# utiasASRL/mm_masking

Measured on AMD Instinct MI355X. Metric: scan-pairs/s (mask-CNN + 10-iter dICP fwd+bwd), higher is better.
Workload: dtype bf16; 1 GPU; BASELINE configs[2]: train_icp_weights step fwd+bwd, batch=32 per GPU, 10 dICP iters, point-to-plane Huber, dim=2; 400x3360 polar radar -> GO-CFAR + peaks + polar->Cartesian 640x640 -> U-Net (hand-written NHWC bf16 MFMA kernels, fp32 masters) -> dICP (fp32 points, fp64 normal equations) -> rot+trans+mask_pts loss -> Adam; batch_per_gpu=32, global_batch=32, scan_pts_pad=5120, map_pts=20000, map_pts_pad=20480, icp_iters=10, parallelism=dp1, scene_density=survey (SURVEY.md 8d: 3 500-5 000 valid scan points of 5 120)

## Files before the change

mm_masking_amd/csrc/mmk_unet.hip:

```cpp
#include <math.h>
#include <stdlib.h>

#include <algorithm>
#include <type_traits>

#include "mmk_common.h"
#include "mmk_unet_shared.h"

namespace {

using namespace mmku;

__device__ __forceinline__ unsigned cvt_pk_bf16(float lo, float hi)
{
    unsigned r;
    asm("v_cvt_pk_bf16_f32 %0, %1, %2" : "=v"(r) : "v"(lo), "v"(hi));
    return r;
}
__device__ __forceinline__ unsigned pk_relu_bf16(unsigned x)
{
    unsigned r;
    asm("v_pk_max_i16 %0, %1, 0" : "=v"(r) : "v"(x));
    return r;
}
// ... 412 lines not shown
    return __builtin_bit_cast(u32x4, o);
}

__device__ __forceinline__ void lds_barrier()
{
    asm volatile("s_waitcnt lgkmcnt(0)\n\ts_barrier" ::: "memory");
}

__device__ __forceinline__ u32x4 poolg_scale(const u32x4 g, float scale)
{
    float f[8];
    unpack8(g, f);
#pragma unroll
    for (int j = 0; j < 8; ++j) f[j] = f[j] * scale;
    return pack8(f);
}
template <int K>
__device__ __forceinline__ u32x4 poolg_route(const u32x4 v, unsigned code)
{
    const unsigned x = code ^ ((unsigned)(K | 4) * 0x11111111u);
    const unsigned t = x | (x >> 1) | (x >> 2);
    const unsigned te = t << 7, to = t << 3;
    u32x4 o;
#pragma unroll
    for (int j = 0; j < 4; ++j) {
        unsigned m;
        asm("v_pk_ashrrev_i16 %0, %1, %2" : "=v"(m) : "v"(0x000f000fu), "v"(__builtin_amdgcn_perm(to, te, 0x040c000cu + (unsigned)j * 0x01000100u)));
        o[j] = v[j] & ~m;
    }
    return o;
}
__device__ __forceinline__ void poolg_write(bf16 *dst, int pitch, int row, int r0, int c0, int rows, int cols, bool on,
                                            const u32x4 g, unsigned code, float scale)
{
    const u32x4 v = poolg_scale(g, scale);
    const bool r_lo = on && (unsigned)r0 < (unsigned)rows, r_hi = on && (unsigned)(r0 + 1) < (unsigned)rows;
    const bool c_lo = (unsigned)c0 < (unsigned)cols, c_hi = (unsigned)(c0 + 1) < (unsigned)cols;
    if (r_lo && c_lo) *reinterpret_cast<u32x4 *>(dst) = poolg_route<0>(v, code);
    if (r_lo && c_hi) *reinterpret_cast<u32x4 *>(dst + pitch) = poolg_route<1>(v, code);
    if (r_hi && c_lo) *reinterpret_cast<u32x4 *>(dst + row) = poolg_route<2>(v, code);
    if (r_hi && c_hi) *reinterpret_cast<u32x4 *>(dst + row + pitch) = poolg_route<3>(v, code);
}

#ifdef MMK_DEEP_STAMPS
constexpr int MMK_STAMP_STAGES = 24;
__device__ unsigned long long *g_deep_stamp_buf = nullptr;
#define MMK_STAMP(K)                                                                                          \
    do {                                                                                                      \
        if (stamp_stage < MMK_STAMP_STAGES) {                                                                 \
            const unsigned long long t_ = __builtin_amdgcn_s_memtime();                                       \
            if (lane == 0) stamp_lds[(wv * MMK_STAMP_STAGES + stamp_stage) * 8 + (K)] = t_;                    \
        }                                                                                                     \
    } while (0)
#else
#define MMK_STAMP(K) do { } while (0)
#endif

#ifndef MMK_RING_DIAG
#define MMK_RING_DIAG 0
#endif
template <int CK, int CM, int RD, bool EPI, int POOL = 0, bool C8 = false, bool POOLG = false>
__global__ __launch_bounds__(CONV_THREADS) void conv3x3_ring_kernel(const ConvArgs a, int total_tiles, int tiles_per_xcd)
{
    static_assert(!(EPI && POOL), "the pooled output belongs to the forward pass (no epilogue operands)");
    static_assert(!C8 || (CM == 16 && !POOL), "C8: a single output part of exactly 8 channels");
    constexpr int NS = ksteps(CK);
    constexpr int MT = CM / 16;
    constexpr int NT = 4;
    constexpr int PK = lds_pitch(CK);
    constexpr int GPP = CK / 8;
    constexpr int NIN = HT * WT * GPP;
    constexpr int NW = NS * MT * 64;
    constexpr int RIN = (NIN + CONV_THREADS - 1) / CONV_THREADS;
    constexpr int RW = (NW + CONV_THREADS - 1) / CONV_THREADS;
    constexpr int NST = C8 ? 1 : (POOL == 2 ? 2 * MT : MT * NT + (POOL ? MT : 0));
    extern __shared__ __attribute__((aligned(16))) unsigned char smem[];
    bf16 *in_tile = reinterpret_cast<bf16 *>(smem);
    bf16 *w_lds = in_tile + 2 * HT * WT * PK;

    const int tid = threadIdx.x, lane = tid & 63, wv = tid >> 6;
    const int tiles_x = (a.W + TW - 1) / TW, tiles_y = (a.H + TH - 1) / TH;
    const int tpi = tiles_x * tiles_y;
    const int group = blockIdx.y;

    const int xcd = blockIdx.x & 7, nb = gridDim.x >> 3;
    const int t_begin = xcd * tiles_per_xcd;
    const int t_end = (t_begin + tiles_per_xcd < total_tiles) ? t_begin + tiles_per_xcd : total_tiles;
    const int first = t_begin + (blockIdx.x >> 3);
    if (first >= t_end) return;
    const int nt_blk = (t_end - first + nb - 1) / nb;
#ifdef MMK_DEEP_STAMPS
    unsigned long long *stamp_lds = reinterpret_cast<unsigned long long *>(smem + ((size_t)(2 * HT * WT * PK + NS * MT * 512) * sizeof(bf16) + 15) / 16 * 16);
    int stamp_stage = 0;
    for (int i = tid; i < 4 * MMK_STAMP_STAGES * 8; i += CONV_THREADS) stamp_lds[i] = 0ull;
    __syncthreads();
    if (tid == 0) {
        stamp_lds[6] = gridDim.x; stamp_lds[7] = (unsigned long long)nt_blk;
        stamp_lds[8 + 6] = __builtin_amdgcn_s_memtime(); stamp_lds[8 + 7] = __builtin_amdgcn_s_memrealtime();
    }
#endif

    constexpr int PHT = TH / 2 + 2, PWT = TW / 2 + 2, NPIN = PHT * PWT * GPP;
    constexpr int NRIN = POOLG ? (NPIN + CONV_THREADS - 1) / CONV_THREADS : RIN;
    u32x4 rin[RD][NRIN];
    unsigned rcd[POOLG ? RD : 1][POOLG ? NRIN : 1];
    int g_dy[RIN], g_dx[RIN], in_off[RIN];
    bool in_x2[RIN];
#pragma unroll
// ... 1057 lines not shown
            }
        } else {
#pragma unroll
        for (int i = 0; i < RG; ++i) {
            int gi = tv + i * CONV_THREADS;
            gi = gi < NG ? gi : NG - 1;
            const int pix = gi / GPG, gc = gi % GPG;
            const int dy = pix / TW, dx = pix % TW;
            const bool ok = ty0 + dy < a.H && tx0 + dx < a.W;
            const int p = pix0 + dy * a.W + dx;
            const u32x4 *sp = ok ? reinterpret_cast<const u32x4 *>(a.g + ((long)p * a.COUT + group * CM + gc * 8)) : &g_zero16;
            rg[i] = *sp;
        }
        }
    };
    auto store_tile = [&]() {
        int tv = tid;
        asm volatile("" : "+v"(tv));
#pragma unroll
        for (int i = 0; i < RIN; ++i) {
            const int gi = tv + i * CONV_THREADS;
            if (gi < NIN) *reinterpret_cast<u32x4 *>(x_tile + (size_t)(gi / GPP) * PK + (gi % GPP) * 8) = rin[i];
        }
        if constexpr (POOLG) {
#pragma unroll
            for (int i = 0; i < NRG; ++i) {
                const int gi = tv + i * CONV_THREADS;
                const int pp = gi / GPG, gc = gi % GPG;
                const int r0 = 2 * (pp / PWG), c0 = 2 * (pp % PWG);
                poolg_write(g_tile + (r0 * TW + c0) * PG + gc * 8, PG, TW * PG, r0, c0, TH, TW, gi < NPG, rg[i], rc[i], a.g_scale);
            }
        } else {
#pragma unroll
        for (int i = 0; i < RG; ++i) {
            const int gi = tv + i * CONV_THREADS;
            if (gi < NG) *reinterpret_cast<u32x4 *>(g_tile + (size_t)(gi / GPG) * PG + (gi % GPG) * 8) = rg[i];
        }
        }
    };

    int t_first, t_step, t_end;
    if ((gridDim.x & 7) == 0) {
        const int per_xcd = (total_tiles + 7) / 8;
        const int xcd = blockIdx.x & 7;
        t_first = xcd * per_xcd + ((int)blockIdx.x >> 3);
        t_step = (int)gridDim.x >> 3;
        t_end = min(total_tiles, (xcd + 1) * per_xcd);
    } else {
        t_first = blockIdx.x; t_step = gridDim.x; t_end = total_tiles;
    }
    const int adv_tx = t_step % tiles_x, adv_ty = (t_step / tiles_x) % tiles_y, adv_b = t_step / tpi;
    int ld_b = t_first / tpi, ld_ty = (t_first % tpi) / tiles_x, ld_tx = t_first % tiles_x;
    if (t_first < t_end) load_tile(ld_b, ld_ty, ld_tx);
    for (int t = t_first; t < t_end; t += t_step) {
        __syncthreads();
        store_tile();
        __syncthreads();
        {
            if (t + t_step < t_end) {
                ld_tx += adv_tx;
                const int cx = ld_tx >= tiles_x ? 1 : 0;
                ld_tx -= cx ? tiles_x : 0;
                ld_ty += adv_ty + cx;
                const int cy = ld_ty >= tiles_y ? 1 : 0;
                ld_ty -= cy ? tiles_y : 0;
                ld_b += adv_b + cy;
            }
            load_tile(ld_b, ld_ty, ld_tx);
        }
        i32x2 fa[2][2 * MT], fb[2][2 * NTW];
#define WG_ISSUE(R, BUF)                                                                                 \
    {                                                                                                    \
        _Pragma("unroll") for (int m = 0; m < MT; ++m) {                                                 \
            fa[BUF][2 * m] = (m == 0) ? tr_read_o<((R) * TW * PG) * 2>(g_ad)                             \
                           : (m == 1) ? tr_read_o<((R) * TW * PG + 16) * 2>(g_ad)                        \
                           : (m == 2) ? tr_read_o<((R) * TW * PG + 32) * 2>(g_ad)                        \
                                      : tr_read_o<((R) * TW * PG + 48) * 2>(g_ad);                       \
            fa[BUF][2 * m + 1] = (m == 0) ? tr_read_o<((R) * TW * PG + 16 * PG) * 2>(g_ad)                \
                               : (m == 1) ? tr_read_o<((R) * TW * PG + 16 + 16 * PG) * 2>(g_ad)           \
                               : (m == 2) ? tr_read_o<((R) * TW * PG + 32 + 16 * PG) * 2>(g_ad)           \
                                          : tr_read_o<((R) * TW * PG + 48 + 16 * PG) * 2>(g_ad);          \
        }                                                                                                \
        _Pragma("unroll") for (int n = 0; n < NTW; ++n) {                                                \
            fb[BUF][2 * n] = tr_read_o<((R) * WT * PK) * 2>(b_ad[n]);                                    \
            fb[BUF][2 * n + 1] = tr_read_o<((R) * WT * PK + 16 * PK) * 2>(b_ad[n]);                       \
        }                                                                                                \
    }
#define WG_CONSUME(BUF)                                                                                  \
    {                                                                                                    \
        _Pragma("unroll") for (int m = 0; m < MT; ++m) {                                                 \
            const bf16x8 af = frag_from(fa[BUF][2 * m], fa[BUF][2 * m + 1]);                             \
             \
             \
            _Pragma("unroll") for (int n = 0; n < NTW; ++n)                                              \
                acc[m][n] = __builtin_amdgcn_mfma_f32_16x16x32_bf16(af, frag_from(fb[BUF][2 * n], fb[BUF][2 * n + 1]), acc[m][n], 0, 0, 0); \
            accb[m] = __builtin_amdgcn_mfma_f32_16x16x32_bf16(af, ones, accb[m], 0, 0, 0);               \
        }                                                                                                \
    }
#define WG_STEP(R)                                                                                       \
    {                                                                                                    \
        asm volatile("s_waitcnt lgkmcnt(0)" ::: "memory");                                               \
        __builtin_amdgcn_sched_barrier(0);                                                               \
        if ((R) + 1 < TH) WG_ISSUE(((R) + 1 < TH ? (R) + 1 : 0), ((R) + 1) & 1);                         \
        __builtin_amdgcn_sched_barrier(0);                                                               \
        WG_CONSUME((R) & 1);                                                                             \
    }
        WG_ISSUE(0, 0);
        WG_STEP(0) WG_STEP(1) WG_STEP(2) WG_STEP(3) WG_STEP(4) WG_STEP(5) WG_STEP(6) WG_STEP(7)
        static_assert(TH == 8, "WG_STEP expansion above covers 8 tile rows");
#undef WG_STEP
#undef WG_CONSUME
#undef WG_ISSUE
    }

    const size_t pstride = (size_t)9 * a.COUT * a.CIN + a.COUT;
#pragma unroll
    for (int m = 0; m < MT; ++m) {
#pragma unroll
        for (int rr = 0; rr < 4; ++rr) {
            const int co = group * CM + m * 16 + g4 * 4 + rr;
            if (co >= a.COUT) continue;
#pragma unroll
            for (int n = 0; n < NTW; ++n) {
                const int nt = wv + 4 * n;
                if (nt >= NTT) continue;
                int tap, ci;
                if (CK >= 16) {
                    tap = nt / (CK / 16);
                    ci = chunk * CK + (nt % (CK / 16)) * 16 + i16;
                } else {
                    tap = 2 * nt + (i16 >> 3);
                    ci = i16 & 7;
                }
                if (tap < 9) {
                    float *d = a.partials + (size_t)blockIdx.x * pstride + ((size_t)tap * a.COUT + co) * a.CIN + ci;
                    *d = a.acc_partials ? *d + acc[m][n][rr] : acc[m][n][rr];
                }
            }
            if (wv == 0 && chunk == 0 && i16 == 0) {
                float *d = a.partials + (size_t)blockIdx.x * pstride + (size_t)9 * a.COUT * a.CIN + co;
                *d = a.acc_partials ? *d + accb[m][rr] : accb[m][rr];
            }
        }
    }
}

constexpr size_t wgrad_smem(int CX, int CG)
{
    return ((size_t)(HT * WT + 8) * wg_pitch(CX) + (size_t)(TH * TW + 8) * wg_pitch(CG)) * sizeof(bf16);
}

template <int CK, int CM, bool G8>
int wgrad_spatial(int cout, int cin, int B, int H, int W)
{
    constexpr int cap = (CK <= 16 && CM == 16) ? 4 : 8;
    int per_cu = 0;
    if (blocks_per_cu<conv3x3_wgrad_kernel<CK, CM, G8>>(CONV_THREADS, wgrad_smem(CK, G8 ? 8 : CM), cap, &per_cu) != hipSuccess) return -1;
    const int tiles = ((W + TW - 1) / TW) * ((H + TH - 1) / TH) * B;
    const int chunks = cin / CK, groups = (cout + CM - 1) / CM;
    int spatial = (256 * per_cu) / (chunks * groups);
    spatial = spatial < 1 ? 1 : (spatial > tiles ? tiles : spatial);
    return spatial >= 8 ? (spatial & ~7) : spatial;
}

template <int CK, int CM, bool G8, bool POOLG = false>
// ... 334 lines not shown
            float *d = a.partials + (size_t)blockIdx.x * pstride + (size_t)9 * CG * CX + co;
            *d = a.acc_partials ? *d + accb[rr] : accb[rr];
        }
    }
}

constexpr int WGD_THREADS = 512;

template <bool POOLG = false>
__global__ __launch_bounds__(WGD_THREADS) void conv3x3_wgrad_deep_kernel(const WgradArgs a)
{
    constexpr int CK = 64, CM = 64, PK = wg_pitch(64), PG = wg_pitch(64);
    extern __shared__ __attribute__((aligned(16))) unsigned char smem[];
    bf16 *x_tile = reinterpret_cast<bf16 *>(smem);
    bf16 *g_tile = x_tile + (HT * WT + 8) * PK;

    const int tid = threadIdx.x, lane = tid & 63;
    const int wv = __builtin_amdgcn_readfirstlane(tid >> 6);
    const int wm = wv >> 2, wc = wv & 3;
    const int chunk = blockIdx.y, group = blockIdx.z;
    const int tiles_x = (a.W + TW - 1) / TW, tiles_y = (a.H + TH - 1) / TH;
    const int tpi = tiles_x * tiles_y;
    const int total_tiles = tpi * a.B;
    const int i16 = lane & 15, g4 = lane >> 4, q = i16 >> 2, pp = i16 & 3;

    f32x4 acc[3][3][2];
    f32x4 accb[2];
#pragma unroll
    for (int m = 0; m < 2; ++m) {
        accb[m] = (f32x4){0.f, 0.f, 0.f, 0.f};
#pragma unroll
        for (int ty = 0; ty < 3; ++ty)
#pragma unroll
            for (int tx = 0; tx < 3; ++tx) acc[ty][tx][m] = (f32x4){0.f, 0.f, 0.f, 0.f};
    }
    bf16x8 ones;
#pragma unroll
    for (int j = 0; j < 8; ++j) ones[j] = (bf16)1.0f;

    const unsigned xb0 = lds_addr(x_tile) + (unsigned)(((4 * g4 + q) * PK + wc * 16 + 4 * pp) * 2);
    const unsigned gb0 = lds_addr(g_tile) + (unsigned)(((4 * g4 + q) * PG + wm * 32 + 4 * pp) * 2);

    constexpr int GPP = CK / 8;
    constexpr int NIN = HT * WT * GPP;
    constexpr int RIN = (NIN + WGD_THREADS - 1) / WGD_THREADS;
    constexpr int GPG = CM / 8;
    constexpr int NG = TH * TW * GPG;
    constexpr int RG = (NG + WGD_THREADS - 1) / WGD_THREADS;
    constexpr int PWG = TW / 2, NPG = (TH / 2) * PWG * GPG;
    constexpr int NRG = POOLG ? (NPG + WGD_THREADS - 1) / WGD_THREADS : RG;
    u32x4 rin[RIN], rg[NRG];
    unsigned rc[POOLG ? NRG : 1];
    const int Hp = a.H >> 1, Wp = a.W >> 1;
    auto load_tile = [&](int b, int tyi, int txi) {
        int tv = tid;
        asm volatile("" : "+v"(tv));
        const int tx0 = txi * TW, ty0 = tyi * TH;
        const int c0 = chunk * CK;
        const bool in1 = c0 < a.C1;
        const bf16 *xb = in1 ? a.x1 : a.x2;
        const int xc = in1 ? a.C1 : a.C2, cb = in1 ? c0 : c0 - a.C1;
#pragma unroll
        for (int i = 0; i < RIN; ++i) {
            int gi = tv + i * WGD_THREADS;
            gi = gi < NIN ? gi : NIN - 1;
            const int pix = gi / GPP, gc = gi % GPP;
            const int yy = ty0 + pix / WT - 1, xx = tx0 + pix % WT - 1;
            const bool ok = yy >= 0 && yy < a.H && xx >= 0 && xx < a.W;
            const size_t p = ((size_t)b * a.H + yy) * a.W + xx;
            const u32x4 *sp = ok ? reinterpret_cast<const u32x4 *>(xb + p * xc + cb + gc * 8) : &g_zero16;
            rin[i] = *sp;
        }
        if constexpr (POOLG) {
#pragma unroll
            for (int i = 0; i < NRG; ++i) {
                int gi = tv + i * WGD_THREADS;
                gi = gi < NPG ? gi : NPG - 1;
                const int pp = gi / GPG, gc = gi % GPG;
                const int py = (ty0 >> 1) + pp / PWG, px = (tx0 >> 1) + pp % PWG;
                const bool ok = py < Hp && px < Wp;
                const size_t e = (((size_t)b * Hp + py) * Wp + px) * (a.COUT >> 3) + ((group * CM) >> 3) + gc;
                rg[i] = *(ok ? reinterpret_cast<const u32x4 *>(a.g + e * 8) : &g_zero16);
                rc[i] = *(ok ? a.g_arg + e : reinterpret_cast<const unsigned *>(&g_zero16));
            }
        } else {
#pragma unroll
        for (int i = 0; i < RG; ++i) {
            int gi = tv + i * WGD_THREADS;
            gi = gi < NG ? gi : NG - 1;
            const int pix = gi / GPG, gc = gi % GPG;
            const int yy = ty0 + pix / TW, xx = tx0 + pix % TW;
            const bool ok = yy < a.H && xx < a.W;
            const size_t p = ((size_t)b * a.H + yy) * a.W + xx;
            const u32x4 *sp = ok ? reinterpret_cast<const u32x4 *>(a.g + p * a.COUT + group * CM + gc * 8) : &g_zero16;
            rg[i] = *sp;
        }
        }
    };
    auto store_tile = [&]() {
        int tv = tid;
        asm volatile("" : "+v"(tv));
#pragma unroll
        for (int i = 0; i < RIN; ++i) {
            const int gi = tv + i * WGD_THREADS;
            if (gi < NIN) *reinterpret_cast<u32x4 *>(x_tile + (size_t)(gi / GPP) * PK + (gi % GPP) * 8) = rin[i];
        }
        if constexpr (POOLG) {
#pragma unroll
            for (int i = 0; i < NRG; ++i) {
                const int gi = tv + i * WGD_THREADS;
                const int pp = gi / GPG, gc = gi % GPG;
                const int r0 = 2 * (pp / PWG), c0 = 2 * (pp % PWG);
                poolg_write(g_tile + (r0 * TW + c0) * PG + gc * 8, PG, TW * PG, r0, c0, TH, TW, gi < NPG, rg[i], rc[i], a.g_scale);
            }
        } else {
#pragma unroll
        for (int i = 0; i < RG; ++i) {
            const int gi = tv + i * WGD_THREADS;
            if (gi < NG) *reinterpret_cast<u32x4 *>(g_tile + (size_t)(gi / GPG) * PG + (gi % GPG) * 8) = rg[i];
        }
        }
    };

    int t_first, t_step, t_end;
    if ((gridDim.x & 7) == 0) {
        const int per_xcd = (total_tiles + 7) / 8;
        const int xcd = blockIdx.x & 7;
        t_first = xcd * per_xcd + ((int)blockIdx.x >> 3);
        t_step = (int)gridDim.x >> 3;
        t_end = min(total_tiles, (xcd + 1) * per_xcd);
    } else {
        t_first = blockIdx.x; t_step = gridDim.x; t_end = total_tiles;
    }
    const int adv_tx = t_step % tiles_x, adv_ty = (t_step / tiles_x) % tiles_y, adv_b = t_step / tpi;
    int ld_b = t_first / tpi, ld_ty = (t_first % tpi) / tiles_x, ld_tx = t_first % tiles_x;
    if (t_first < t_end) load_tile(ld_b, ld_ty, ld_tx);
    for (int t = t_first; t < t_end; t += t_step) {
        __syncthreads();
        store_tile();
        __syncthreads();
        {
            if (t + t_step < t_end) {
                ld_tx += adv_tx;
                const int cx = ld_tx >= tiles_x ? 1 : 0;
                ld_tx -= cx ? tiles_x : 0;
                ld_ty += adv_ty + cx;
                const int cy = ld_ty >= tiles_y ? 1 : 0;
                ld_ty -= cy ? tiles_y : 0;
                ld_b += adv_b + cy;
            }
            load_tile(ld_b, ld_ty, ld_tx);
        }
        i32x2 fb[2][3][2], fa[4][2][2];
#define WGD_ISSUE(RHO)                                                                                   \
    {                                                                                                    \
        fb[(RHO) & 1][0][0] = tr_read_o<(((RHO) * WT + 0) * PK) * 2>(xb0);                               \
        fb[(RHO) & 1][0][1] = tr_read_o<(((RHO) * WT + 0) * PK + 16 * PK) * 2>(xb0);                     \
        fb[(RHO) & 1][1][0] = tr_read_o<(((RHO) * WT + 1) * PK) * 2>(xb0);                               \
        fb[(RHO) & 1][1][1] = tr_read_o<(((RHO) * WT + 1) * PK + 16 * PK) * 2>(xb0);                     \
        fb[(RHO) & 1][2][0] = tr_read_o<(((RHO) * WT + 2) * PK) * 2>(xb0);                               \
        fb[(RHO) & 1][2][1] = tr_read_o<(((RHO) * WT + 2) * PK + 16 * PK) * 2>(xb0);                     \
        if ((RHO) < TH) {                                                                                \
            constexpr int R_ = (RHO) < TH ? (RHO) : 0;                                                   \
            fa[R_ & 3][0][0] = tr_read_o<((R_ * TW) * PG) * 2>(gb0);                                     \
            fa[R_ & 3][0][1] = tr_read_o<((R_ * TW) * PG + 16 * PG) * 2>(gb0);                           \
            fa[R_ & 3][1][0] = tr_read_o<((R_ * TW) * PG + 16) * 2>(gb0);                                \
            fa[R_ & 3][1][1] = tr_read_o<((R_ * TW) * PG + 16 + 16 * PG) * 2>(gb0);                      \
        }                                                                                                \
    }
#define WGD_STEP(RHO)                                                                                    \
    {                                                                                                    \
        asm volatile("s_waitcnt lgkmcnt(0)" ::: "memory");                                               \
        __builtin_amdgcn_sched_barrier(0);                                                               \
                                          \
        if ((RHO) + 1 < HT) WGD_ISSUE(((RHO) + 1 < HT ? (RHO) + 1 : 0));                                 \
        __builtin_amdgcn_sched_barrier(0);                                                               \
        bf16x8 bfr[3];                                                                                   \
        _Pragma("unroll") for (int tx = 0; tx < 3; ++tx) bfr[tx] = frag_from(fb[(RHO) & 1][tx][0], fb[(RHO) & 1][tx][1]); \
        _Pragma("unroll") for (int ty = 0; ty < 3; ++ty) {                                               \
            const int r = (RHO) - ty;                \
            if (r >= 0 && r < TH) {                                                                      \
                _Pragma("unroll") for (int m = 0; m < 2; ++m) {                                          \
                    const bf16x8 af = frag_from(fa[r & 3][m][0], fa[r & 3][m][1]);                       \
                    _Pragma("unroll") for (int tx = 0; tx < 3; ++tx)                                     \
                        acc[ty][tx][m] = __builtin_amdgcn_mfma_f32_16x16x32_bf16(af, bfr[tx], acc[ty][tx][m], 0, 0, 0); \
                    if (ty == 0) accb[m] = __builtin_amdgcn_mfma_f32_16x16x32_bf16(af, ones, accb[m], 0, 0, 0);  \
                }                                                                                        \
            }                                                                                            \
        }                                                                                                \
        __builtin_amdgcn_sched_barrier(0);                                                               \
    }
        WGD_ISSUE(0);
        WGD_STEP(0) WGD_STEP(1) WGD_STEP(2) WGD_STEP(3) WGD_STEP(4)
        WGD_STEP(5) WGD_STEP(6) WGD_STEP(7) WGD_STEP(8) WGD_STEP(9)
        static_assert(HT == 10, "WGD_STEP expansion above covers 10 halo rows");
#undef WGD_STEP
#undef WGD_ISSUE
    }

    const size_t pstride = (size_t)9 * a.COUT * a.CIN + a.COUT;
#pragma unroll
    for (int m = 0; m < 2; ++m) {
#pragma unroll
        for (int rr = 0; rr < 4; ++rr) {
            const int co = group * CM + (wm * 2 + m) * 16 + g4 * 4 + rr;
            const int ci = chunk * CK + wc * 16 + i16;
            {
                float *ps = a.partials + (size_t)blockIdx.x * pstride + (size_t)co * a.CIN + ci;
#pragma unroll
                for (int ty = 0; ty < 3; ++ty)
#pragma unroll
                    for (int tx = 0; tx < 3; ++tx) {
                        float *d = ps + (size_t)(ty * 3 + tx) * a.COUT * a.CIN;
                        *d = a.acc_partials ? *d + acc[ty][tx][m][rr] : acc[ty][tx][m][rr];
                    }
            }
            if (wc == 0 && chunk == 0 && i16 == 0) {
                float *d = a.partials + (size_t)blockIdx.x * pstride + (size_t)9 * a.COUT * a.CIN + co;
                *d = a.acc_partials ? *d + accb[m][rr] : accb[m][rr];
            }
        }
    }
}

int wgrad_deep_slices(int cout, int cin, int B, int H, int W)
{
    const int tiles = ((W + TW - 1) / TW) * ((H + TH - 1) / TH) * B;
    const int chunks = cin / 64, groups = cout / 64;
    int spatial = 256 / (chunks * groups);
    spatial = spatial < 1 ? 1 : (spatial > tiles ? tiles : spatial);
    return spatial >= 8 ? (spatial & ~7) : spatial;
}

bool wgrad_is_deep(int cout, int cin, int c1) { return cin % 64 == 0 && cout % 64 == 0 && c1 % 64 == 0; }

template <bool POOLG = false>
int launch_wgrad_deep(const WgradArgs &a, hipStream_t st)
{
    constexpr size_t smem = wgrad_smem(64, 64);
    MMK_CHECK_HIP(raise_lds_limit<conv3x3_wgrad_deep_kernel<POOLG>>(true, smem));
    const int spatial = wgrad_deep_slices(a.COUT, a.CIN, a.B, a.H, a.W);
    const int chunks = a.CIN / 64, groups = a.COUT / 64;
    hipLaunchKernelGGL(conv3x3_wgrad_deep_kernel<POOLG>, dim3(spatial, chunks, groups), dim3(WGD_THREADS), smem, st, a);
    MMK_LAUNCH_CHECK();
    return MMK_OK;
}

template <class F>
int with_wgrad_shape(int cout, int cin, F &&f)
{
    return with_int<8, 16, 32, 64>(cin_chunk(cin), [&](auto K) {
        return with_int<16, 32, 64>(cout_group(cout), [&](auto M) {
            if constexpr (M() == 16) {
                if (cout == 8) return f(K, M, std::true_type{});
            }
            return f(K, M, std::false_type{});
        });
    });
}

int dispatch_wgrad(const WgradArgs &a, hipStream_t st)
{
    if (a.g_arg != nullptr) {
        if (wgrad_is_deep(a.COUT, a.CIN, a.C1)) return launch_wgrad_deep<true>(a, st);
        if (a.CIN == 32 && a.COUT == 32) return launch_wgrad<32, 32, false, true>(a, st);
        mmk::set_error("mmk_conv3x3_wgrad_partial_pooled: unsupported channel counts CIN=%d COUT=%d", a.CIN, a.COUT);
        return MMK_ERR_ARG;
    }
    if (wgrad_is_deep(a.COUT, a.CIN, a.C1)) return launch_wgrad_deep(a, st);
    const int rc = with_wgrad_shape(a.COUT, a.CIN, [&](auto K, auto M, auto G8) { return launch_wgrad<K(), M(), G8()>(a, st); });
    if (rc != NO_KERNEL) return rc;
    mmk::set_error("mmk_conv3x3_wgrad: unsupported channel counts CIN=%d COUT=%d", a.CIN, a.COUT);
    return MMK_ERR_ARG;
}

int wgrad_slices(int cout, int cin, int c1, int B, int H, int W)
{
    if (wgrad_is_deep(cout, cin, c1)) return wgrad_deep_slices(cout, cin, B, H, W);
    const int ns = with_wgrad_shape(cout, cin, [&](auto K, auto M, auto G8) { return wgrad_spatial<K(), M(), G8()>(cout, cin, B, H, W); });
    return ns == NO_KERNEL ? 0 : ns;
}

struct UnpackBatch {
    const float *src[PACK_BATCH_MAX];
    float *dW[PACK_BATCH_MAX];
    float *db[PACK_BATCH_MAX];
    int cout[PACK_BATCH_MAX], cin[PACK_BATCH_MAX], slices[PACK_BATCH_MAX];
};

__host__ __device__ inline int unpack_groups(int total) { return total < 8192 ? 16 : (total < 65536 ? 4 : 1); }

__global__ __launch_bounds__(256) void unpack_wgrad_batch_kernel(const UnpackBatch ub)
// ... 255 lines not shown
#pragma unroll
            for (int px = 0; px < 4; ++px) {
                bf16x8 o;
#pragma unroll
                for (int co = 0; co < 8; ++co) o[co] = (bf16)(LK ? act_leaky(acc[px][co], slope) : fmaxf(acc[px][co], 0.f));
                *reinterpret_cast<bf16x8 *>(dst + px * 8) = o;
            }
#pragma unroll
            for (int dy = 0; dy < 3; ++dy)
#pragma unroll
                for (int i = 0; i < 6; ++i) rv[dy][i] = rn[dy][i];
            mv = mn;
        }
        return;
    }
    for (int e = blockIdx.x * blockDim.x + threadIdx.x; e < nq; e += gridDim.x * blockDim.x) {
        const int q = e % Wq, by = e / Wq;
        const int yy = by % H, b = by / H;
        const int x0 = q * 4;
        float acc[4][8];
#pragma unroll
        for (int px = 0; px < 4; ++px)
#pragma unroll
            for (int co = 0; co < 8; ++co) acc[px][co] = bs[co];
        for (int c = 0; c < CIN; ++c) {
            const float *xc = x + ((size_t)b * CIN + c) * H * W;
            const float psub = pre ? pre[2 * c] : 0.f, prcp = pre ? pre[2 * c + 1] : 1.f;
#pragma unroll
            for (int dy = 0; dy < 3; ++dy) {
                float v[6];
                load_row6(xc, yy + dy - 1, x0, H, W, psub, prcp, v);
#pragma unroll
                for (int co = 0; co < 8; ++co) {
#pragma unroll
                    for (int tx = 0; tx < 3; ++tx) {
                        const float w = Wt[(co * CIN + c) * 9 + dy * 3 + tx];
#pragma unroll
                        for (int px = 0; px < 4; ++px) acc[px][co] = __builtin_fmaf(v[px + tx], w, acc[px][co]);
                    }
                }
            }
        }
        bf16 *dst = y + ((size_t)by * W + x0) * 8;
#pragma unroll
        for (int px = 0; px < 4; ++px) {
            bf16x8 o;
#pragma unroll
            for (int co = 0; co < 8; ++co) o[co] = (bf16)(LK ? act_leaky(acc[px][co], slope) : fmaxf(acc[px][co], 0.f));
            *reinterpret_cast<bf16x8 *>(dst + px * 8) = o;
        }
    }
}

__global__ __launch_bounds__(256) void conv_first_wgrad_x4_kernel(const float *__restrict__ x, int CIN, const bf16 *__restrict__ g,
                                                                  const float *__restrict__ pre, int B, int H, int W,
                                                                  float *__restrict__ part )
{
    __shared__ float red[4][80];
    const int lane = threadIdx.x & 63, wv = threadIdx.x >> 6;
    const int Wq = W >> 2;
    const int nq = B * H * Wq;
    const int stride = gridDim.x * blockDim.x;
    for (int c = 0; c < CIN; ++c) {
        const float psub = pre ? pre[2 * c] : 0.f, prcp = pre ? pre[2 * c + 1] : 1.f;
        float acc[80];
#pragma unroll
        for (int i = 0; i < 80; ++i) acc[i] = 0.f;
        bf16x8 gv[4], gn[4];
        float rv[3][6], rn[3][6];
        unsigned mv = 0, mn = 0;
        auto fetch = [&](int e, bf16x8 (&go)[4], float (&ro)[3][6], unsigned &mo) {
            const int q = e % Wq, by = e / Wq;
            const int yy = by % H, b = by / H;
            const int x0 = q * 4;
            const float *xc = x + ((size_t)b * CIN + c) * H * W;
            const bf16 *gp = g + ((size_t)by * W + x0) * 8;
#pragma unroll
            for (int px = 0; px < 4; ++px) go[px] = *reinterpret_cast<const bf16x8 *>(gp + px * 8);
            unsigned m = 0;
#pragma unroll
            for (int dy = 0; dy < 3; ++dy) {
                const int y2 = yy + dy - 1;
                const bool rok = y2 >= 0 && y2 < H;
                const float *row = xc + (size_t)(rok ? y2 : yy) * W;
                const bool lok = x0 > 0, hok = x0 + 4 < W;
                const float4 mid = *reinterpret_cast<const float4 *>(row + x0);
                ro[dy][0] = row[lok ? x0 - 1 : x0];
                ro[dy][1] = mid.x; ro[dy][2] = mid.y; ro[dy][3] = mid.z; ro[dy][4] = mid.w;
                ro[dy][5] = row[hok ? x0 + 4 : x0 + 3];
                m |= (rok ? ((lok ? 1u : 0u) | 0x1Eu | (hok ? 0x20u : 0u)) : 0u) << (6 * dy);
            }
            mo = m;
        };
        int e = blockIdx.x * blockDim.x + threadIdx.x;
        if (e < nq) fetch(e, gv, rv, mv);
        for (; e < nq; e += stride) {
            const int en = e + stride;
            fetch(en < nq ? en : e, gn, rn, mn);
            float v[3][6];
#pragma unroll
            for (int dy = 0; dy < 3; ++dy)
#pragma unroll
                for (int i = 0; i < 6; ++i) {
                    const float t = (rv[dy][i] - psub) * prcp;
                    v[dy][i] = ((mv >> (6 * dy + i)) & 1u) ? (float)(bf16)t : 0.f;
                }
// ... 1290 lines not shown
        const int nblk = (int)std::min<int64_t>(BN_BLOCKS, (npix + per - 1) / per);
        hipLaunchKernelGGL(bn_bwd_reduce_kernel, dim3(nblk), dim3(256), 0, st, (const bf16 *)gd, (const bf16 *)d, drop_scale,
                           (const bf16 *)a, (size_t)npix, C, stat, part);
        MMK_LAUNCH_CHECK();
        hipLaunchKernelGGL(bn_bwd_finalize_kernel, dim3((C + 63) / 64), dim3(64), 0, st, part, nblk, C, (double)npix, gamma, stat,
                           accumulate, coef, dgamma, dbeta);
        MMK_LAUNCH_CHECK();
    } else {
        MMK_REQUIRE(affine != nullptr, "mmk_bn_backward: evaluation mode needs the affine (scale, shift) pairs");
        hipLaunchKernelGGL(bn_eval_coef_kernel, dim3((C + 63) / 64), dim3(64), 0, st, affine, C, coef);
        MMK_LAUNCH_CHECK();
    }
    hipLaunchKernelGGL(bn_bwd_apply_kernel, dim3(gb), dim3(256), 0, st, (const bf16 *)gd, (const bf16 *)d, drop_scale, (const bf16 *)a,
                       ngran, C, stat, coef, leaky_slope, (bf16 *)gz);
    MMK_LAUNCH_CHECK();
    return MMK_OK;
}

static unsigned nblk(size_t n, int t) { return (unsigned)((n + t - 1) / t); }

extern "C" int mmk_channel_minmax(const float *x, int32_t B, int32_t C, int64_t hw, float *part, float *pre, float *minmax,
                                  void *stream)
{
    MMK_REQUIRE(x && part && pre && B >= 1 && C >= 1 && C <= 65535 && hw >= 1, "mmk_channel_minmax: bad argument");
    hipStream_t st = (hipStream_t)stream;
    hipLaunchKernelGGL(channel_minmax_partial_kernel, dim3(MM_BLOCKS, C), dim3(256), 0, st, x, B, C, (size_t)hw, part);
    MMK_LAUNCH_CHECK();
    hipLaunchKernelGGL(channel_minmax_final_kernel, dim3(C), dim3(256), 0, st, part, C, pre, minmax);
    MMK_LAUNCH_CHECK();
    return MMK_OK;
}

extern "C" int mmk_channel_meanstd(const float *x, int32_t B, int32_t C, int64_t hw, double *part, float *pre, void *stream)
{
    MMK_REQUIRE(x && part && pre && B >= 1 && C >= 1 && C <= 65535 && hw >= 1, "mmk_channel_meanstd: bad argument");
    hipStream_t st = (hipStream_t)stream;
    hipLaunchKernelGGL(channel_moment_partial_kernel<false>, dim3(MM_BLOCKS, C), dim3(256), 0, st, x, B, C, (size_t)hw, part);
    MMK_LAUNCH_CHECK();
    hipLaunchKernelGGL(channel_moment_partial_kernel<true>, dim3(MM_BLOCKS, C), dim3(256), 0, st, x, B, C, (size_t)hw, part);
    MMK_LAUNCH_CHECK();
    hipLaunchKernelGGL(channel_meanstd_final_kernel, dim3(C), dim3(256), 0, st, (const double *)part, (size_t)B * (size_t)hw, pre);
    MMK_LAUNCH_CHECK();
    return MMK_OK;
}

extern "C" int mmk_conv_first(const float *x, int32_t cin, const float *W, const float *bias, const float *pre, int32_t B,
                              int32_t H, int32_t Wd, float leaky_slope, void *y, void *stream)
{
    MMK_REQUIRE(x && W && y, "mmk_conv_first: NULL pointer");
    MMK_REQUIRE(leaky_slope >= 0.f && leaky_slope < 1.f, "mmk_conv_first: leaky_slope must be in [0, 1)");
    MMK_REQUIRE(cin >= 1 && cin <= 4 && B >= 1 && H >= 1 && Wd >= 1, "mmk_conv_first: bad shape (cin must be 1..4)");
    const size_t npix = (size_t)B * H * Wd;
    if (Wd % 4 == 0 && npix < (1u << 31)) {
        const unsigned blocks = (unsigned)std::min<size_t>((npix / 4 + 255) / 256, 4096);
        if (leaky_slope > 0.f)
            hipLaunchKernelGGL(conv_first_x4_kernel<true>, dim3(blocks), dim3(256), 0, (hipStream_t)stream, x, cin, W, bias, pre, B, H, Wd,
                               leaky_slope, (bf16 *)y);
        else
            hipLaunchKernelGGL(conv_first_x4_kernel<false>, dim3(blocks), dim3(256), 0, (hipStream_t)stream, x, cin, W, bias, pre, B, H, Wd,
                               leaky_slope, (bf16 *)y);
        MMK_LAUNCH_CHECK();
        return MMK_OK;
    }
    const unsigned blocks = (unsigned)std::min<size_t>((npix + 255) / 256, 8192);
    hipLaunchKernelGGL(conv_first_kernel, dim3(blocks), dim3(256), 0, (hipStream_t)stream, x, cin, W, bias, pre, B, H, Wd, leaky_slope,
                       (bf16 *)y);
    MMK_LAUNCH_CHECK();
    return MMK_OK;
}

extern "C" size_t mmk_conv_first_wgrad_ws_bytes(int32_t cin) { return (size_t)1024 * (cin < 1 ? 1 : cin) * 80 * sizeof(float); }

extern "C" int mmk_conv_first_wgrad(const float *x, int32_t cin, const void *g, const float *pre, int32_t B, int32_t H,
                                    int32_t Wd, float *dW, float *db, float *ws, size_t ws_bytes, void *stream)
{
    MMK_REQUIRE(x && g && dW && ws, "mmk_conv_first_wgrad: NULL pointer");
    MMK_REQUIRE(cin >= 1 && cin <= 4 && B >= 1 && H >= 1 && Wd >= 1, "mmk_conv_first_wgrad: bad shape");
    MMK_REQUIRE(ws_bytes >= mmk_conv_first_wgrad_ws_bytes(cin), "mmk_conv_first_wgrad: workspace too small (%zu < %zu bytes)", ws_bytes,
                mmk_conv_first_wgrad_ws_bytes(cin));
    const size_t npix = (size_t)B * H * Wd;
    unsigned blocks;
    if (Wd % 4 == 0 && npix < (1u << 31)) {
        blocks = (unsigned)std::min<size_t>((npix / 4 + 255) / 256, 512);
        hipLaunchKernelGGL(conv_first_wgrad_x4_kernel, dim3(blocks), dim3(256), 0, (hipStream_t)stream, x, cin, (const bf16 *)g, pre,
                           B, H, Wd, ws);
    } else {
        blocks = (unsigned)std::min<size_t>((npix + 255) / 256, 1024);
        hipLaunchKernelGGL(conv_first_wgrad_kernel, dim3(blocks), dim3(256), 0, (hipStream_t)stream, x, cin, (const bf16 *)g, pre, B,
                           H, Wd, ws);
    }
    MMK_LAUNCH_CHECK();
    hipLaunchKernelGGL(conv_first_wgrad_reduce_kernel, dim3(cin), dim3(320), 0, (hipStream_t)stream, ws, (int)blocks, cin, dW, db);
    MMK_LAUNCH_CHECK();
    return MMK_OK;
}

extern "C" size_t mmk_conv_first_dgrad_ws_bytes(int32_t cin)
{
    return (size_t)(cin < 1 ? 1 : cin) * 4 * (1 + DG_BLOCKS) * sizeof(double);
}

namespace {
template <int CIN, int MODE>
void launch_first_dgrad(bool tiled, unsigned blocks, hipStream_t st, const bf16 *g, const float *W, const float *x, const float *pre,
                        const float *minmax, int B, int H, int Wd, float *gx, double *part)
{
// ... 227 lines not shown
```

Before: 3422 pairs/s.

## Interleave deep wgrad next-tile global loads with the MFMA row steps

The deep weight-gradient kernel's next-tile prefetch no longer issues every global load in one block right after the barrier. Each load is now issued one at a time inside the per-halo-row MFMA steps, with precomputed tile base pointers and unsigned 32-bit address math. The aim is to spread memory traffic across the compute loop, hide latency, and cut address-calculation overhead. The change also adds stamp-based timing instrumentation behind MMK_DEEP_STAMPS, which is compiled out by default, and the tail guards now fold at compile time.

```diff
diff --git a/mm_masking_amd/csrc/mmk_unet.hip b/mm_masking_amd/csrc/mmk_unet.hip
--- a/mm_masking_amd/csrc/mmk_unet.hip
+++ b/mm_masking_amd/csrc/mmk_unet.hip
@@ -488,8 +488,16 @@
             if (lane == 0) stamp_lds[(wv * MMK_STAMP_STAGES + stamp_stage) * 8 + (K)] = t_;                    \
         }                                                                                                     \
     } while (0)
+#define MMK_STAMP_G(K)                                                                                        \
+    do {                                                                                                      \
+        if (stamp_on && stamp_stage < MMK_STAMP_STAGES) {                                                     \
+            const unsigned long long t_ = __builtin_amdgcn_s_memtime();                                       \
+            if (lane == 0) g_deep_stamp_buf[((size_t)(blockIdx.x * 8 + wv) * MMK_STAMP_STAGES + stamp_stage) * 8 + (K)] = t_; \
+        }                                                                                                     \
+    } while (0)
 #else
 #define MMK_STAMP(K) do { } while (0)
+#define MMK_STAMP_G(K) do { } while (0)
 #endif
 
 #ifndef MMK_RING_DIAG
@@ -1653,10 +1661,22 @@
     const int adv_tx = t_step % tiles_x, adv_ty = (t_step / tiles_x) % tiles_y, adv_b = t_step / tpi;
     int ld_b = t_first / tpi, ld_ty = (t_first % tpi) / tiles_x, ld_tx = t_first % tiles_x;
     if (t_first < t_end) load_tile(ld_b, ld_ty, ld_tx);
+#ifdef MMK_DEEP_STAMPS
+    const bool stamp_on = g_deep_stamp_buf != nullptr && blockIdx.x < 64 && blockIdx.y == 0 && blockIdx.z == 0;
+    int stamp_stage = 0;
+#endif
     for (int t = t_first; t < t_end; t += t_step) {
+        MMK_STAMP_G(0);
         __syncthreads();
+        MMK_STAMP_G(1);
+#ifdef MMK_DEEP_STAMPS
+        asm volatile("s_waitcnt vmcnt(0)" ::: "memory");
+#endif
+        MMK_STAMP_G(2);
         store_tile();
+        MMK_STAMP_G(3);
         __syncthreads();
+        MMK_STAMP_G(4);
         {
             if (t + t_step < t_end) {
                 ld_tx += adv_tx;
@@ -1669,6 +1689,7 @@
             }
             load_tile(ld_b, ld_ty, ld_tx);
         }
+        MMK_STAMP_G(5);
         i32x2 fa[2][2 * MT], fb[2][2 * NTW];
 #define WG_ISSUE(R, BUF)                                                                                 \
     {                                                                                                    \
@@ -1707,11 +1728,17 @@
         WG_CONSUME((R) & 1);                                                                             \
     }
         WG_ISSUE(0, 0);
-        WG_STEP(0) WG_STEP(1) WG_STEP(2) WG_STEP(3) WG_STEP(4) WG_STEP(5) WG_STEP(6) WG_STEP(7)
+        WG_STEP(0)
+        MMK_STAMP_G(6);
+        WG_STEP(1) WG_STEP(2) WG_STEP(3) WG_STEP(4) WG_STEP(5) WG_STEP(6) WG_STEP(7)
         static_assert(TH == 8, "WG_STEP expansion above covers 8 tile rows");
 #undef WG_STEP
 #undef WG_CONSUME
 #undef WG_ISSUE
+        MMK_STAMP_G(7);
+#ifdef MMK_DEEP_STAMPS
+        ++stamp_stage;
+#endif
     }
 
     const size_t pstride = (size_t)9 * a.COUT * a.CIN + a.COUT;
@@ -2152,49 +2179,61 @@
     u32x4 rin[RIN], rg[NRG];
     unsigned rc[POOLG ? NRG : 1];
     const int Hp = a.H >> 1, Wp = a.W >> 1;
-    auto load_tile = [&](int b, int tyi, int txi) {
-        int tv = tid;
+    constexpr int NLD = RIN + (POOLG ? 2 * NRG : RG);
+    static_assert(NLD <= HT, "one prefetch load per row step");
+    const int c0 = chunk * CK;
+    const bool in1 = c0 < a.C1;
+    const bf16 *xb = in1 ? a.x1 : a.x2;
+    const int xc = in1 ? a.C1 : a.C2, cb = in1 ? c0 : c0 - a.C1;
+    const bf16 *ld_x = nullptr, *ld_g = nullptr;
+    const unsigned *ld_c = nullptr;
+    int ld_ty0 = 0, ld_tx0 = 0;
+    typedef const __attribute__((address_space(1))) u32x4 *gvec_p;
+    typedef const __attribute__((address_space(1))) unsigned *gword_p;
+    gvec_p zero16 = (gvec_p)&g_zero16;
+    asm volatile("" : "+s"(zero16));
+    auto set_tile = [&](int b, int tyi, int txi) {
+        ld_tx0 = txi * TW;
+        ld_ty0 = tyi * TH;
+        ld_x = xb + (((long)b * a.H + ld_ty0 - 1) * a.W + ld_tx0 - 1) * xc + cb;
+        if constexpr (POOLG) {
+            const long e = (((long)b * Hp + (ld_ty0 >> 1)) * Wp + (ld_tx0 >> 1)) * (a.COUT >> 3) + ((group * CM) >> 3);
+            ld_g = a.g + e * 8;
+            ld_c = a.g_arg + e;
+        } else {
+            ld_g = a.g + (((long)b * a.H + ld_ty0) * a.W + ld_tx0) * a.COUT + group * CM;
+        }
+    };
+    auto issue_load = [&](int j) {
+        unsigned tv = (unsigned)tid;
         asm volatile("" : "+v"(tv));
-        const int tx0 = txi * TW, ty0 = tyi * TH;
-        const int c0 = chunk * CK;
-        const bool in1 = c0 < a.C1;
-        const bf16 *xb = in1 ? a.x1 : a.x2;
-        const int xc = in1 ? a.C1 : a.C2, cb = in1 ? c0 : c0 - a.C1;
-#pragma unroll
-        for (int i = 0; i < RIN; ++i) {
-            int gi = tv + i * WGD_THREADS;
-            gi = gi < NIN ? gi : NIN - 1;
-            const int pix = gi / GPP, gc = gi % GPP;
-            const int yy = ty0 + pix / WT - 1, xx = tx0 + pix % WT - 1;
-            const bool ok = yy >= 0 && yy < a.H && xx >= 0 && xx < a.W;
-            const size_t p = ((size_t)b * a.H + yy) * a.W + xx;
-            const u32x4 *sp = ok ? reinterpret_cast<const u32x4 *>(xb + p * xc + cb + gc * 8) : &g_zero16;
-            rin[i] = *sp;
-        }
-        if constexpr (POOLG) {
-#pragma unroll
-            for (int i = 0; i < NRG; ++i) {
-                int gi = tv + i * WGD_THREADS;
-                gi = gi < NPG ? gi : NPG - 1;
-                const int pp = gi / GPG, gc = gi % GPG;
-                const int py = (ty0 >> 1) + pp / PWG, px = (tx0 >> 1) + pp % PWG;
-                const bool ok = py < Hp && px < Wp;
-                const size_t e = (((size_t)b * Hp + py) * Wp + px) * (a.COUT >> 3) + ((group * CM) >> 3) + gc;
-                rg[i] = *(ok ? reinterpret_cast<const u32x4 *>(a.g + e * 8) : &g_zero16);
-                rc[i] = *(ok ? a.g_arg + e : reinterpret_cast<const unsigned *>(&g_zero16));
-            }
+        if (j < RIN) {
+            unsigned gi = tv + (unsigned)(j * WGD_THREADS);
+            gi = gi < (unsigned)NIN ? gi : (unsigned)(NIN - 1);
+            const unsigned pix = gi / GPP, gc = gi % GPP;
+            const unsigned row = pix / WT, col = pix % WT;
+            const bool ok = ((unsigned)(ld_ty0 - 1) + row < (unsigned)a.H) & ((unsigned)(ld_tx0 - 1) + col < (unsigned)a.W);
+            const unsigned off = (row * (unsigned)a.W + col) * (unsigned)xc + gc * 8;
+            rin[j] = *(ok ? (gvec_p)(ld_x + off) : zero16);
+        } else if constexpr (POOLG) {
+            const int i = (j - RIN) % NRG;
+            unsigned gi = tv + (unsigned)(i * WGD_THREADS);
+            gi = gi < (unsigned)NPG ? gi : (unsigned)(NPG - 1);
+            const unsigned pp = gi / GPG, gc = gi % GPG;
+            const unsigned pr = pp / PWG, pc = pp % PWG;
+            const bool ok = ((unsigned)(ld_ty0 >> 1) + pr < (unsigned)Hp) & ((unsigned)(ld_tx0 >> 1) + pc < (unsigned)Wp);
+            const unsigned e = (pr * (unsigned)Wp + pc) * (unsigned)(a.COUT >> 3) + gc;
+            if (j - RIN < NRG) rg[i] = *(ok ? (gvec_p)(ld_g + e * 8) : zero16);
+            else rc[i] = *(ok ? (gword_p)(ld_c + e) : (gword_p)zero16);
         } else {
-#pragma unroll
-        for (int i = 0; i < RG; ++i) {
-            int gi = tv + i * WGD_THREADS;
-            gi = gi < NG ? gi : NG - 1;
-            const int pix = gi / GPG, gc = gi % GPG;
-            const int yy = ty0 + pix / TW, xx = tx0 + pix % TW;
-            const bool ok = yy < a.H && xx < a.W;
-            const size_t p = ((size_t)b * a.H + yy) * a.W + xx;
-            const u32x4 *sp = ok ? reinterpret_cast<const u32x4 *>(a.g + p * a.COUT + group * CM + gc * 8) : &g_zero16;
-            rg[i] = *sp;
-        }
+            const int i = j - RIN;
+            unsigned gi = tv + (unsigned)(i * WGD_THREADS);
+            gi = gi < (unsigned)NG ? gi : (unsigned)(NG - 1);
+            const unsigned pix = gi / GPG, gc = gi % GPG;
+            const unsigned row = pix / TW, col = pix % TW;
+            const bool ok = ((unsigned)ld_ty0 + row < (unsigned)a.H) & ((unsigned)ld_tx0 + col < (unsigned)a.W);
+            const unsigned off = (row * (unsigned)a.W + col) * (unsigned)a.COUT + gc * 8;
+            rg[i] = *(ok ? (gvec_p)(ld_g + off) : zero16);
         }
     };
     auto store_tile = [&]() {
@@ -2203,7 +2242,7 @@
 #pragma unroll
         for (int i = 0; i < RIN; ++i) {
             const int gi = tv + i * WGD_THREADS;
-            if (gi < NIN) *reinterpret_cast<u32x4 *>(x_tile + (size_t)(gi / GPP) * PK + (gi % GPP) * 8) = rin[i];
+            if ((i + 1) * WGD_THREADS <= NIN || gi < NIN) *reinterpret_cast<u32x4 *>(x_tile + (size_t)(gi / GPP) * PK + (gi % GPP) * 8) = rin[i];
         }
         if constexpr (POOLG) {
 #pragma unroll
@@ -2211,13 +2250,14 @@
                 const int gi = tv + i * WGD_THREADS;
                 const int pp = gi / GPG, gc = gi % GPG;
                 const int r0 = 2 * (pp / PWG), c0 = 2 * (pp % PWG);
-                poolg_write(g_tile + (r0 * TW + c0) * PG + gc * 8, PG, TW * PG, r0, c0, TH, TW, gi < NPG, rg[i], rc[i], a.g_scale);
+                poolg_write(g_tile + (r0 * TW + c0) * PG + gc * 8, PG, TW * PG, r0, c0, TH, TW, (i + 1) * WGD_THREADS <= NPG || gi < NPG, rg[i],
+                            rc[i], a.g_scale);
             }
         } else {
 #pragma unroll
         for (int i = 0; i < RG; ++i) {
             const int gi = tv + i * WGD_THREADS;
-            if (gi < NG) *reinterpret_cast<u32x4 *>(g_tile + (size_t)(gi / GPG) * PG + (gi % GPG) * 8) = rg[i];
+            if ((i + 1) * WGD_THREADS <= NG || gi < NG) *reinterpret_cast<u32x4 *>(g_tile + (size_t)(gi / GPG) * PG + (gi % GPG) * 8) = rg[i];
         }
         }
     };
@@ -2234,11 +2274,29 @@
     }
     const int adv_tx = t_step % tiles_x, adv_ty = (t_step / tiles_x) % tiles_y, adv_b = t_step / tpi;
     int ld_b = t_first / tpi, ld_ty = (t_first % tpi) / tiles_x, ld_tx = t_first % tiles_x;
-    if (t_first < t_end) load_tile(ld_b, ld_ty, ld_tx);
+    if (t_first < t_end) {
+        set_tile(ld_b, ld_ty, ld_tx);
+#pragma unroll
+        for (int j = 0; j < NLD; ++j) issue_load(j);
+    }
+#ifdef MMK_DEEP_STAMPS
+    unsigned long long *stamp_lds = reinterpret_cast<unsigned long long *>(smem + (wgrad_smem(64, 64) + 15) / 16 * 16);
+    int stamp_stage = 0;
+    for (int i = tid; i < 8 * MMK_STAMP_STAGES * 8; i += WGD_THREADS) stamp_lds[i] = 0ull;
+    __syncthreads();
+#endif
     for (int t = t_first; t < t_end; t += t_step) {
+        MMK_STAMP(0);
         __syncthreads();
+        MMK_STAMP(1);
+#ifdef MMK_DEEP_STAMPS
+        asm volatile("s_waitcnt vmcnt(0)" ::: "memory");
+#endif
+        MMK_STAMP(2);
         store_tile();
+        MMK_STAMP(3);
         __syncthreads();
+        MMK_STAMP(4);
         {
             if (t + t_step < t_end) {
                 ld_tx += adv_tx;
@@ -2249,8 +2307,9 @@
                 ld_ty -= cy ? tiles_y : 0;
                 ld_b += adv_b + cy;
             }
-            load_tile(ld_b, ld_ty, ld_tx);
-        }
+            set_tile(ld_b, ld_ty, ld_tx);
+        }
+        MMK_STAMP(5);
         i32x2 fb[2][3][2], fa[4][2][2];
 #define WGD_ISSUE(RHO)                                                                                   \
     {                                                                                                    \
@@ -2275,6 +2334,9 @@
                                           \
         if ((RHO) + 1 < HT) WGD_ISSUE(((RHO) + 1 < HT ? (RHO) + 1 : 0));                                 \
         __builtin_amdgcn_sched_barrier(0);                                                               \
+                                                                                \
+        if ((RHO) < NLD) issue_load((RHO) < NLD ? (RHO) : 0);                                            \
+        __builtin_amdgcn_sched_barrier(0x38F);                                                           \
         bf16x8 bfr[3];                                                                                   \
         _Pragma("unroll") for (int tx = 0; tx < 3; ++tx) bfr[tx] = frag_from(fb[(RHO) & 1][tx][0], fb[(RHO) & 1][tx][1]); \
         _Pragma("unroll") for (int ty = 0; ty < 3; ++ty) {                                               \
@@ -2284,19 +2346,32 @@
                     const bf16x8 af = frag_from(fa[r & 3][m][0], fa[r & 3][m][1]);                       \
                     _Pragma("unroll") for (int tx = 0; tx < 3; ++tx)                                     \
                         acc[ty][tx][m] = __builtin_amdgcn_mfma_f32_16x16x32_bf16(af, bfr[tx], acc[ty][tx][m], 0, 0, 0); \
-                    if (ty == 0) accb[m] = __builtin_amdgcn_mfma_f32_16x16x32_bf16(af, ones, accb[m], 0, 0, 0);  \
+                     \
+                    if (ty == 0) accb[m] = __builtin_amdgcn_mfma_f32_16x16x32_bf16(af, ones, accb[m], 0, 0, 0); \
                 }                                                                                        \
             }                                                                                            \
         }                                                                                                \
         __builtin_amdgcn_sched_barrier(0);                                                               \
     }
         WGD_ISSUE(0);
-        WGD_STEP(0) WGD_STEP(1) WGD_STEP(2) WGD_STEP(3) WGD_STEP(4)
+        WGD_STEP(0)
+        MMK_STAMP(6);
+        WGD_STEP(1) WGD_STEP(2) WGD_STEP(3) WGD_STEP(4)
         WGD_STEP(5) WGD_STEP(6) WGD_STEP(7) WGD_STEP(8) WGD_STEP(9)
         static_assert(HT == 10, "WGD_STEP expansion above covers 10 halo rows");
 #undef WGD_STEP
 #undef WGD_ISSUE
-    }
+        MMK_STAMP(7);
+#ifdef MMK_DEEP_STAMPS
+        ++stamp_stage;
+#endif
+    }
+#ifdef MMK_DEEP_STAMPS
+    __syncthreads();
+    if (g_deep_stamp_buf != nullptr && blockIdx.y == 0 && blockIdx.z == 0 && blockIdx.x < 64)
+        for (int i = tid; i < 8 * MMK_STAMP_STAGES * 8; i += WGD_THREADS)
+            g_deep_stamp_buf[(size_t)blockIdx.x * (8 * MMK_STAMP_STAGES * 8) + i] = stamp_lds[i];
+#endif
 
     const size_t pstride = (size_t)9 * a.COUT * a.CIN + a.COUT;
 #pragma unroll
@@ -2337,7 +2412,11 @@
 template <bool POOLG = false>
 int launch_wgrad_deep(const WgradArgs &a, hipStream_t st)
 {
+#ifdef MMK_DEEP_STAMPS
+    constexpr size_t smem = (wgrad_smem(64, 64) + 15) / 16 * 16 + (size_t)8 * MMK_STAMP_STAGES * 8 * sizeof(unsigned long long);
+#else
     constexpr size_t smem = wgrad_smem(64, 64);
+#endif
     MMK_CHECK_HIP(raise_lds_limit<conv3x3_wgrad_deep_kernel<POOLG>>(true, smem));
     const int spatial = wgrad_deep_slices(a.COUT, a.CIN, a.B, a.H, a.W);
     const int chunks = a.CIN / 64, groups = a.COUT / 64;
```

Result: faster. 3467 pairs/s, median of 6 (+1.3%).

## Add row-band first-conv kernel with sliding window and LDS-transposed coalesced stores

Applied to the files above, without the earlier changes.

Adds a specialised first-convolution kernel for the single-channel, ReLU case. Each thread walks a vertical band of 8 rows with a sliding 3-row register window, so each input row is loaded once instead of three times. Output is reshuffled through a swizzled LDS buffer within each wavefront so global bf16x8 stores become contiguous across lanes. It is on by default with an environment opt-out, and it launches one thread per band-column, which means fewer threads and more serial work per thread.

```diff
diff --git a/mm_masking_amd/csrc/mmk_unet.hip b/mm_masking_amd/csrc/mmk_unet.hip
--- a/mm_masking_amd/csrc/mmk_unet.hip
+++ b/mm_masking_amd/csrc/mmk_unet.hip
@@ -2699,6 +2699,108 @@
     }
 }
 
+constexpr int CF_BAND = 8;
+
+__global__ __launch_bounds__(256) void conv_first_band_kernel(const float *__restrict__ x, const float *__restrict__ Wt,
+                                                              const float *__restrict__ bias, const float *__restrict__ pre, int B,
+                                                              int H, int W, bf16 *__restrict__ y)
+{
+    __shared__ u32x4 xch[4][256];
+    float bs[8];
+#pragma unroll
+    for (int co = 0; co < 8; ++co) bs[co] = bias ? bias[co] : 0.f;
+    const float psub = pre ? pre[0] : 0.f, prcp = pre ? pre[1] : 1.f;
+    const int lane = threadIdx.x & 63, wv = threadIdx.x >> 6;
+    const int Wq = W >> 2;
+    const int nb = (H + CF_BAND - 1) / CF_BAND;
+    const int n_items = B * nb * Wq;
+    const int item_raw = blockIdx.x * blockDim.x + threadIdx.x;
+    const bool valid = item_raw < n_items;
+    const int item = valid ? item_raw : n_items - 1;
+    const int q = item % Wq, t = item / Wq;
+    const int band = t % nb, b = t / nb;
+    const int x0 = q * 4;
+    const int y0 = band * CF_BAND;
+    const int my_rows = valid ? min(H, y0 + CF_BAND) - y0 : 0;
+    const int my_pix = (b * H + y0) * W + x0;
+    int own_pix[4], own_rows[4];
+#pragma unroll
+    for (int k = 0; k < 4; ++k) {
+        own_pix[k] = __shfl(my_pix, k * 16 + (lane >> 2), 64) + (lane & 3);
+        own_rows[k] = __shfl(my_rows, k * 16 + (lane >> 2), 64);
+    }
+    const float *xc = x + (size_t)b * H * W;
+    const bool lok = x0 > 0, hok = x0 + 4 < W;
+    auto fetch = [&](int y2, float (&ro)[6]) {
+        const float *row = xc + (size_t)min(max(y2, 0), H - 1) * W;
+        const float4 mid = *reinterpret_cast<const float4 *>(row + x0);
+        ro[0] = row[lok ? x0 - 1 : x0];
+        ro[1] = mid.x; ro[2] = mid.y; ro[3] = mid.z; ro[4] = mid.w;
+        ro[5] = row[hok ? x0 + 4 : x0 + 3];
+    };
+    auto finish = [&](int y2, const float (&ro)[6], float (&v)[6]) {
+        const bool rok = y2 >= 0 && y2 < H;
+#pragma unroll
+        for (int i = 0; i < 6; ++i) {
+            const float tv = (ro[i] - psub) * prcp;
+            const bool ok = rok && (i != 0 || lok) && (i != 5 || hok);
+            v[i] = ok ? (float)(bf16)tv : 0.f;
+        }
+    };
+    float win[3][6], raw[6];
+    fetch(y0 - 1, raw);
+    finish(y0 - 1, raw, win[0]);
+    fetch(y0, raw);
+    finish(y0, raw, win[1]);
+    fetch(y0 + 1, raw);
+    for (int s = 0; s < CF_BAND; ++s) {
+        if (__ballot(s < my_rows) == 0) break;
+        const int yy = y0 + s;
+        finish(yy + 1, raw, win[2]);
+        fetch(yy + 2, raw);
+        float acc[4][8];
+#pragma unroll
+        for (int px = 0; px < 4; ++px)
+#pragma unroll
+            for (int co = 0; co < 8; ++co) acc[px][co] = bs[co];
+#pragma unroll
+        for (int dy = 0; dy < 3; ++dy)
+#pragma unroll
+            for (int co = 0; co < 8; ++co)
+#pragma unroll
+                for (int tx = 0; tx < 3; ++tx) {
+                    const float w = Wt[co * 9 + dy * 3 + tx];
+#pragma unroll
+                    for (int px = 0; px < 4; ++px) acc[px][co] = __builtin_fmaf(win[dy][px + tx], w, acc[px][co]);
+                }
+        bf16x8 o[4];
+#pragma unroll
+        for (int px = 0; px < 4; ++px)
+#pragma unroll
+            for (int co = 0; co < 8; ++co) o[px][co] = (bf16)fmaxf(acc[px][co], 0.f);
+        u32x4 *xw = xch[wv];
+#pragma unroll
+        for (int px = 0; px < 4; ++px) xw[lane * 4 + (px ^ ((lane >> 2) & 3))] = __builtin_bit_cast(u32x4, o[px]);
+        __builtin_amdgcn_fence(__ATOMIC_RELEASE, "wavefront");
+        __builtin_amdgcn_wave_barrier();
+        __builtin_amdgcn_fence(__ATOMIC_ACQUIRE, "wavefront");
+#pragma unroll
+        for (int k = 0; k < 4; ++k) {
+            const int P = k * 64 + lane;
+            const u32x4 v = xw[(P & ~3) | ((P & 3) ^ ((P >> 4) & 3))];
+            if (s < own_rows[k]) *reinterpret_cast<u32x4 *>(y + ((size_t)own_pix[k] + (size_t)s * W) * 8) = v;
+        }
+        __builtin_amdgcn_fence(__ATOMIC_RELEASE, "wavefront");
+        __builtin_amdgcn_wave_barrier();
+        __builtin_amdgcn_fence(__ATOMIC_ACQUIRE, "wavefront");
+#pragma unroll
+        for (int i = 0; i < 6; ++i) {
+            win[0][i] = win[1][i];
+            win[1][i] = win[2][i];
+        }
+    }
+}
+
 __global__ __launch_bounds__(256) void conv_first_wgrad_x4_kernel(const float *__restrict__ x, int CIN, const bf16 *__restrict__ g,
                                                                   const float *__restrict__ pre, int B, int H, int W,
                                                                   float *__restrict__ part )
@@ -4095,6 +4197,14 @@
     MMK_REQUIRE(cin >= 1 && cin <= 4 && B >= 1 && H >= 1 && Wd >= 1, "mmk_conv_first: bad shape (cin must be 1..4)");
     const size_t npix = (size_t)B * H * Wd;
     if (Wd % 4 == 0 && npix < (1u << 31)) {
+        const char *tiled_env = getenv("MMK_CONV_FIRST_TILED");
+        if (cin == 1 && leaky_slope == 0.f && !(tiled_env && tiled_env[0] == '0')) {
+            const size_t items = (size_t)B * ((H + CF_BAND - 1) / CF_BAND) * (Wd / 4);
+            hipLaunchKernelGGL(conv_first_band_kernel, dim3((unsigned)((items + 255) / 256)), dim3(256), 0, (hipStream_t)stream, x, W, bias,
+                               pre, B, H, Wd, (bf16 *)y);
+            MMK_LAUNCH_CHECK();
+            return MMK_OK;
+        }
         const unsigned blocks = (unsigned)std::min<size_t>((npix / 4 + 255) / 256, 4096);
         if (leaky_slope > 0.f)
             hipLaunchKernelGGL(conv_first_x4_kernel<true>, dim3(blocks), dim3(256), 0, (hipStream_t)stream, x, cin, W, bias, pre, B, H, Wd,
```

New measurement: 3549 pairs/s before, 3555 pairs/s after (median of 6 runs). No clear change (+0.2%).
